# tpfeifle/pointcloud-segmentation-attention

Hardware: AMD Instinct MI355X
Metric: 8192-pt clouds/sec through SA+FP layers, 1/2/4/8 MI355X; HBM GB/s vs peak (higher is better)
Workload: dtype f32

## Files before the change

### include/pn2hip.h

```cpp
#ifndef PN2HIP_H
#define PN2HIP_H

#include <stddef.h>
#include <stdint.h>

#ifdef __cplusplus
extern "C" {
#endif

typedef void* pn2_stream_t;

#define PN2_OK 0
#define PN2_EINVAL (-22)
#define PN2_EFAULT (-14)
#define PN2_ENOTSUP (-95)

#define PN2_FAULT_FPS_POLL 1

#define PN2_FPS_AUTO 0
#define PN2_FPS_BLOCKSCAN 1

#define PN2_USE_XYZ 1
#define PN2_XYZ_LAST 2

// ... 90 lines not shown
  const float* new_xyz;
  int N, C, M, nsample;
  float radius;
  int flags;
  int32_t* idx;
  int32_t* pts_cnt;
  float* grouped_xyz;
  float* new_points;
} pn2_sa_layer;
int pn2_ball_group_layers(const pn2_sa_layer* layers, int nlayers, int B, pn2_stream_t stream);


int pn2_three_nn(const float* xyz1, const float* xyz2, int B, int n, int m, float* dist,
                 int32_t* idx, pn2_stream_t stream);
int pn2_three_interpolate(const float* points, const int32_t* idx, const float* weight, int B,
                          int m, int C, int n, float* out, pn2_stream_t stream);
int pn2_three_interpolate_grad(const float* grad_out, const int32_t* idx, const float* weight,
                               int B, int n, int C, int m, float* grad_points,
                               pn2_stream_t stream);
int pn2cpu_three_nn(const float* xyz1, const float* xyz2, int B, int n, int m, float* dist,
                    int32_t* idx);
int pn2cpu_three_interpolate(const float* points, const int32_t* idx, const float* weight, int B,
                             int m, int C, int n, float* out);
int pn2cpu_three_interpolate_grad(const float* grad_out, const int32_t* idx, const float* weight,
                                  int B, int n, int C, int m, float* grad_points);
int pn2_idw_weights(const float* dist, int B, int n, float* weight, pn2_stream_t stream);
int pn2_fp_fused(const float* xyz1, const float* xyz2, const float* points1, int C1,
                 const float* points2, int C2, int B, int n, int m, float* out,
                 pn2_stream_t stream);

#define PN2_FP_MAX_LAYERS 4
typedef struct pn2_fp_layer {
  const float* xyz1;
  const float* xyz2;
  const float* points1;
  const float* points2;
  int C1, C2, n, m;
  float* out;
} pn2_fp_layer;
int pn2_fp_fused_layers(const pn2_fp_layer* layers, int nlayers, int B, pn2_stream_t stream);

int pn2_three_nn_grid(const void* known_grid, const void* unknown_grid, const float* xyz1,
                      int B, int n, int m, float* dist, int32_t* idx, pn2_stream_t stream);
int pn2_fp_apply(const float* dist, const int32_t* idx, const void* unknown_grid,
                 const float* points1, int C1, const float* points2, int C2, int B, int n, int m,
                 float* out, pn2_stream_t stream);
int pn2_fp_grid_fused(const float* xyz1, const float* xyz2, const void* unknown_grid,
                      const float* points1, int C1, const float* points2, int C2, int B, int n,
                      int m, float* out, float* dist, int32_t* idx, pn2_stream_t stream);
int pn2_fp_grid_fused_known(const void* known_grid, const float* xyz1, const float* xyz2,
                            const void* unknown_grid, const float* points1, int C1,
                            const float* points2, int C2, int B, int n, int m, float* out,
                            float* dist, int32_t* idx, pn2_stream_t stream);


int pn2_attn_reduce(const float* Q, const float* K, const float* V, int B, int M, int ns,
                    int C, float* out, pn2_stream_t stream);
#define PN2_ATTN_MAX_LAYERS 4
typedef struct pn2_attn_layer {
  const float* Q;
  const float* K;
  const float* V;
  int M, ns, C;
  float* out;
} pn2_attn_layer;
int pn2_attn_reduce_layers(const pn2_attn_layer* layers, int nlayers, int B,
                           pn2_stream_t stream);
int pn2_attn_reduce_grad(const float* Q, const float* K, const float* V, const float* grad_out,
                         int B, int M, int ns, int C, float* grad_Q, float* grad_K,
                         float* grad_V, pn2_stream_t stream);
int pn2_group_pool(const float* x, const float* grouped_xyz, int B, int M, int ns, int C,
                   int mode, float* out, pn2_stream_t stream);


size_t pn2_mlp_packed_size(int cin, int cout);
int pn2_mlp_pack(const float* weight, const float* bias, const float* bn_scale,
                 const float* bn_shift, int cin, int cout, void* packed, size_t packed_bytes,
                 pn2_stream_t stream);

int pn2_group_mlp(const float* xyz, const float* points, const float* new_xyz,
                  const int32_t* idx, int B, int N, int C, int M, int nsample, int flags,
                  int nlayers, const pn2_mlp_layer* layers, int pool, float* out,
                  pn2_stream_t stream);
int pn2_group_mlp_attention(const float* xyz, const float* points, const float* new_xyz,
                            const int32_t* idx, int B, int N, int C, int M, int nsample,
                            int flags, int nlayers, const pn2_mlp_layer* layers,
                            const pn2_mlp_layer* qkv, const float* bn_scale,
                            const float* bn_shift, int add_max, float* out,
                            pn2_stream_t stream);
int pn2_fp_mlp(const float* dist, const int32_t* nn_idx, const float* points1, int C1,
               const float* points2, int C2, int B, int n, int m, int nlayers,
               const pn2_mlp_layer* layers, float* out, pn2_stream_t stream);
int pn2_shared_mlp(const float* x, long long rows, int cin, int nlayers,
                   const pn2_mlp_layer* layers, float* out, pn2_stream_t stream);
int pn2_shared_mlp_plan(long long rows, int cin, int nlayers, const pn2_mlp_layer* layers,
                        int* row_tiles, int* tiles_per_wg);


#define PN2_BN_BLOCK_ROWS 1024
size_t pn2_bn_workspace_size(long long rows, int C);
int pn2_bn_stats(const float* y, long long rows, int C, float* mean, float* var, void* workspace,
                 size_t workspace_bytes, pn2_stream_t stream);
int pn2_bn_act_fwd(const float* y, long long rows, int C, const float* mean, const float* var,
                   const float* gamma, const float* beta, float eps, int relu, float* out,
                   pn2_stream_t stream);
int pn2_bn_act_bwd(const float* grad_out, const float* y, long long rows, int C,
// ... 42 lines not shown
```

### pointcloud-segmentation-attention_amd/_lib.py

```python
import ctypes
import os

import torch

_HERE = os.path.dirname(os.path.abspath(__file__))
LIB_PATH = os.environ.get("PN2HIP_LIB") or os.path.join(_HERE, "libpn2hip.so")

PN2_EINVAL = -22
PN2_BQ_MAX_RADII = 3
PN2_EFAULT = -14
PN2_FAULT_FPS_POLL = 1
PN2_ENOTSUP = -95
PN2_FPS_AUTO, PN2_FPS_BLOCKSCAN = 0, 1
PN2_USE_XYZ = 1
PN2_XYZ_LAST = 2
POOL_MODES = {"max": 0, "avg": 1, "weighted_avg": 2, "max_and_avg": 3}
PN2_POOL_NONE = -1
PN2_MLP_MAX_LAYERS = 6
PN2_MLP_RELU = 1


class InvalidArgumentError(ValueError):
    """Raised where the reference's OP_REQUIRES raises tf.errors.InvalidArgumentError."""

# ... 22 lines not shown


class FpLayer(ctypes.Structure):
    _fields_ = [("xyz1", ctypes.c_void_p), ("xyz2", ctypes.c_void_p),
                ("points1", ctypes.c_void_p), ("points2", ctypes.c_void_p), ("C1", ctypes.c_int),
                ("C2", ctypes.c_int), ("n", ctypes.c_int), ("m", ctypes.c_int),
                ("out", ctypes.c_void_p)]


PN2_FP_MAX_LAYERS = 4


class AttnLayer(ctypes.Structure):
    _fields_ = [("Q", ctypes.c_void_p), ("K", ctypes.c_void_p), ("V", ctypes.c_void_p),
                ("M", ctypes.c_int), ("ns", ctypes.c_int), ("C", ctypes.c_int),
                ("out", ctypes.c_void_p)]


PN2_ATTN_MAX_LAYERS = 4

SIGNATURES = {
    "pn2_version": (ctypes.c_char_p, []),
    "pn2_strerror": (ctypes.c_char_p, [_I]),
    "pn2_copy_f4": (_I, [_P, _P, _S, _I, _P]),
    "pn2_fps": (_I, [_P, _I, _I, _I, _P, _P]),
    "pn2_fps_gather": (_I, [_P, _I, _I, _I, _P, _P, _P]),
    "pn2_fps_max_points": (_I, []),
    "pn2_fps_gather_sched": (_I, [_P, _I, _I, _I, _P, _P, _I, _P]),
    "pn2_fault_status": (_I, [_I]),
    "pn2_prob_sample_workspace_size": (_S, [_I, _I]),
    "pn2_prob_sample": (_I, [_P, _P, _I, _I, _I, _P, _S, _P, _P]),
    "pn2_fps_workspace_size": (_S, [_I, _I]),
    "pn2_fps_chain": (_I, [_P, _I, _I, _I, _P, _P, _P, _P]),
    "pn2_fps_chain_grid": (_I, [_P, _I, _I, _I, _P, _P, _P, _P, _S, _P]),
    "pn2_fps_ws": (_I, [_P, _I, _I, _I, _P, _P, _P, _S, _P]),
    "pn2_gather_point": (_I, [_P, _P, _I, _I, _I, _P, _P]),
    "pn2_gather_point_grad": (_I, [_P, _P, _I, _I, _I, _P, _P]),
    "pn2_ball_query": (_I, [_P, _P, _I, _I, _I, _F, _I, _P, _P, _P]),
    "pn2_ball_threshold": (_F, [_F]),
    "pn2_select_top_k": (_I, [_P, _I, _I, _I, _I, _P, _P, _P, _P]),
    "pn2_select_top_k_workspace_size": (_S, [_I, _I, _I]),
    "pn2_knn_point": (_I, [_P, _P, _I, _I, _I, _I, _I, _P, _P, _P]),
    "pn2_grid_size": (_S, [_I, _I]),
    "pn2_grid_build": (_I, [_P, _I, _I, _F, _P, _S, _P]),
    "pn2_ball_query_grid": (_I, [_P, _P, _I, _I, _I, _F, _I, _P, _P, _P]),
    "pn2_ball_group_xyz_grid": (_I, [_P, _P, _P, _I, _I, _I, _F, _I, _P, _P, _P, _P]),
    "pn2_ball_group_grid": (_I, [_P, _P, _P, _I, _I, _P, _I, _I, _I, _F, _I, _P, _P, _P, _P]),
    "pn2_ball_group_xyz_grid_radii": (_I, [_P, _P, _P, _I, _I, _I, _I, _P, _P, _P, _P, _P, _P]),
    "pn2_three_nn_grid": (_I, [_P, _P, _P, _I, _I, _I, _P, _P, _P]),
    "pn2_fp_apply": (_I, [_P, _P, _P, _P, _I, _P, _I, _I, _I, _I, _P, _P]),
    "pn2_fp_grid_fused": (_I, [_P, _P, _P, _P, _I, _P, _I, _I, _I, _I, _P, _P, _P, _P]),
    "pn2_fp_grid_fused_known": (_I, [_P, _P, _P, _P, _P, _I, _P, _I, _I, _I, _I, _P, _P, _P,
                                     _P]),
    "pn2_group_point": (_I, [_P, _P, _I, _I, _I, _I, _I, _P, _P]),
    "pn2_group_point_grad": (_I, [_P, _P, _I, _I, _I, _I, _I, _P, _P]),
    "pn2_group_concat": (_I, [_P, _P, _P, _P, _I, _I, _I, _I, _I, _I, _P, _P, _P]),
    "pn2_ball_group_layers": (_I, [_P, _I, _I, _P]),
    "pn2_sample_and_group": (_I, [_P, _P, _I, _I, _I, _I, _F, _I, _I, _P, _P, _P, _P, _P, _P,
                                  _P]),
    "pn2_three_nn": (_I, [_P, _P, _I, _I, _I, _P, _P, _P]),
    "pn2_three_interpolate": (_I, [_P, _P, _P, _I, _I, _I, _I, _P, _P]),
    "pn2_three_interpolate_grad": (_I, [_P, _P, _P, _I, _I, _I, _I, _P, _P]),
    "pn2_idw_weights": (_I, [_P, _I, _I, _P, _P]),
    "pn2cpu_three_nn": (_I, [_P, _P, _I, _I, _I, _P, _P]),
    "pn2cpu_three_interpolate": (_I, [_P, _P, _P, _I, _I, _I, _I, _P]),
    "pn2cpu_three_interpolate_grad": (_I, [_P, _P, _P, _I, _I, _I, _I, _P]),
    "pn2_fp_fused_layers": (_I, [_P, _I, _I, _P]),
    "pn2_fp_fused": (_I, [_P, _P, _P, _I, _P, _I, _I, _I, _I, _P, _P]),
    "pn2_attn_reduce": (_I, [_P, _P, _P, _I, _I, _I, _I, _P, _P]),
    "pn2_attn_reduce_layers": (_I, [_P, _I, _I, _P]),
    "pn2_attn_reduce_grad": (_I, [_P, _P, _P, _P, _I, _I, _I, _I, _P, _P, _P, _P]),
    "pn2_group_pool": (_I, [_P, _P, _I, _I, _I, _I, _I, _P, _P]),
    "pn2_mlp_packed_size": (_S, [_I, _I]),
    "pn2_mlp_pack": (_I, [_P, _P, _P, _P, _I, _I, _P, _S, _P]),
    "pn2_group_mlp": (_I, [_P, _P, _P, _P, _I, _I, _I, _I, _I, _I, _I, _P, _I, _P, _P]),
    "pn2_group_mlp_attention": (_I, [_P, _P, _P, _P, _I, _I, _I, _I, _I, _I, _I, _P, _P, _P, _P,
                                     _I, _P, _P]),
    "pn2_fp_mlp": (_I, [_P, _P, _P, _I, _P, _I, _I, _I, _I, _I, _P, _P, _P]),
    "pn2_shared_mlp": (_I, [_P, _LL, _I, _I, _P, _P, _P]),
    "pn2_shared_mlp_plan": (_I, [_LL, _I, _I, _P, _P, _P]),
    "pn2_bn_workspace_size": (_S, [_LL, _I]),
    "pn2_bn_stats": (_I, [_P, _LL, _I, _P, _P, _P, _S, _P]),
    "pn2_bn_act_fwd": (_I, [_P, _LL, _I, _P, _P, _P, _P, _F, _I, _P, _P]),
    "pn2_bn_act_bwd": (_I, [_P, _P, _LL, _I, _P, _P, _P, _P, _F, _I, _P, _P, _P, _P, _S, _P]),
    "pn2_bn_act_pool_fwd": (_I, [_P, _LL, _I, _I, _P, _P, _P, _P, _F, _I, _P, _P, _P]),
    "pn2_bn_pool_workspace_size": (_S, [_LL, _I]),
    "pn2_bn_act_pool_bwd": (_I, [_P, _P, _P, _LL, _I, _I, _P, _P, _P, _P, _F, _I, _P, _P, _P, _P,
                                 _S, _P]),
    "pn2_mlp_wgrad_workspace_size": (_S, [_LL, _I, _I]),
    "pn2_mlp_wgrad": (_I, [_P, _P, _LL, _I, _I, _P, _P, _S, _P]),
    "pn2_scene_workspace_size": (_S, [_I]),
    "pn2_scene_bbox": (_I, [_P, _I, _P, _P, _S, _P]),
    "pn2_crop_workspace_size": (_S, [_I, _I, _I]),
    "pn2_crop_sample": (_I, [_P, _P, _P, _P, _I, _P, _P, _I, _I, _P, _I, _P, _I, _P, _S, _P, _P,
                             _P, _P, _P, _P]),
    "pn2_subvolume_slices": (_I, [_I]),
    "pn2_subvolume_select": (_I, [_P, _I, _P, _I, ctypes.c_double, _P, _P, _P, _P]),
    "pn2_gather_rows": (_I, [_P, _LL, _I, _P, _LL, _P, _P]),
    "pn2_plan_create": (_P, []),
    "pn2_plan_destroy": (None, [_P]),
    "pn2_plan_graph": (_I, [_P, _P, _P]),
    "pn2_plan_record": (_I, [_P, _P, _P]),
    "pn2_plan_wait": (_I, [_P, _P, _P]),
    "pn2_plan_fps_chain": (_I, [_P, _P, _I, _I, _I, _P, _P, _P, _P]),
    "pn2_plan_fps_chain_grid": (_I, [_P, _P, _I, _I, _I, _P, _P, _P, _P, _S, _P]),
    "pn2_plan_mark_timed": (_I, [_P]),
# ... 64 lines not shown
```

### pointcloud-segmentation-attention_amd/csrc/interp.hip

```cpp
#include <algorithm>
#include <type_traits>

#include "grid.h"

namespace pn2 {
namespace {

constexpr int kNNBlock = 256;
constexpr int kNNGroup = 4;
constexpr int kNNRows = kNNBlock / kNNGroup;
constexpr int kNNTile = 2048;

struct Best3 {
  float d1, d2, d3;
  int i1, i2, i3;
};

PN2_DEV void best3_init(Best3& b) {
  b.d1 = b.d2 = b.d3 = __builtin_inff();
  b.i1 = b.i2 = b.i3 = 0;
}

PN2_DEV void best3_insert(Best3& b, float d, int k) {
  const bool c1 = d < b.d1, c2 = d < b.d2, c3 = d < b.d3;
// ... 491 lines not shown
      if (ugrid) jj = __float_as_int(grid_view(ugrid, b, n).pts[jj].w);
      s_row[threadIdx.x] = jj;
      const float* D = pdist + ((size_t)b * n + jj) * 3;
      const int32_t* I = pidx + ((size_t)b * n + jj) * 3;
      float w1, w2, w3;
      idw(D[0], D[1], D[2], w1, w2, w3);
      s_idx[threadIdx.x] = make_int4(I[0], I[1], I[2], 0);
      s_w[threadIdx.x] = make_float4(w1, w2, w3, 0.0f);
    }
  } else {
    const int jl = threadIdx.x / kNNGroup;
    const int j = j0 + jl;
    const bool valid = j < n;
    const float* U = xyz1 + ((size_t)b * n + (valid ? j : 0)) * 3;
    Best3 best;
    best3_init(best);
    scan_known(xyz2 + (size_t)b * m * 3, m, U[0], U[1], U[2], sk, best, tile);
    if ((threadIdx.x & (kNNGroup - 1)) == 0) {
      float w1, w2, w3;
      idw(best.d1, best.d2, best.d3, w1, w2, w3);
      s_idx[jl] = make_int4(best.i1, best.i2, best.i3, 0);
      s_w[jl] = make_float4(w1, w2, w3, 0.0f);
    }
  }
  __syncthreads();
  fp_write_rows<V2, V1, UN>(p, b, zb, j0, [&](int rl) {
    if constexpr (PRE) return FpRow{s_idx[rl], s_w[rl], s_row[rl]};
    else return FpRow{s_idx[rl], s_w[rl], j0 + rl};
  });
}

template <int V2, int V1, bool PRE, int UN>
__global__ __launch_bounds__(kNNBlock) void fp_fused_kernel(FpLayer p, int tile) {
  extern __shared__ float4 sk[];
  const int total = (p.n + kNNRows - 1) / kNNRows * p.B * p.Z;
  const int Lg = xcd_block(blockIdx.x, total);
  if (Lg >= total) return;
  fp_fused_body<V2, V1, PRE, UN>(p, Lg, sk, tile);
}

constexpr int kFpGridMaxKnown = 4096;
constexpr float kFpgPointsPerCell = 2.0f;
constexpr int kFpgBlock = 256;
#ifndef PN2_FPG_STAMP
#define PN2_FPG_STAMP 0
#endif
#if PN2_FPG_STAMP
__device__ unsigned long long g_fpg_stamp[4096 * 8];
#define PN2_FPG_T(K) if (t == 0 && Lg < 4096) g_fpg_stamp[Lg * 8 + (K)] = __builtin_amdgcn_s_memtime();
#else
#define PN2_FPG_T(K)
#endif

size_t device_lds_per_block() {
  static size_t cache[64] = {0};
  int dev = 0;
  if (hipGetDevice(&dev) != hipSuccess || dev < 0 || dev >= 64) return 64 * 1024;
  if (!cache[dev]) {
    int v = 0, o = 0;
    if (hipDeviceGetAttribute(&v, hipDeviceAttributeMaxSharedMemoryPerBlock, dev) != hipSuccess)
      v = 0;
    if (hipDeviceGetAttribute(&o, hipDeviceAttributeSharedMemPerBlockOptin, dev) != hipSuccess)
      o = 0;
    v = std::max(v, o);
    if (v <= 0) return 64 * 1024;
    cache[dev] = (size_t)v;
  }
  return cache[dev];
}

inline size_t fp_grid_lds(int m) {
  const size_t cells = (size_t)ceil((double)m * kAutoPointsPerCell / kFpgPointsPerCell);
  return (size_t)m * 16 + ((std::max(cells, (size_t)kAutoMinCells) + 1) * 2 + 3) / 4 * 4;
}

template <int V2, int V1, int UN, int KPT, int FB>
__global__ __launch_bounds__(FB) void fp_grid_fused_kernel(FpLayer p, float* __restrict__ dist,
                                                        int32_t* __restrict__ idx,
                                                        const char* __restrict__ kgrid) {
  constexpr int NW = FB / kWave;
  constexpr int FR = FB / kNNGroup;
  extern __shared__ float4 s_pts[];
  __shared__ int4 s_idx[FR];
  __shared__ float s_wv[3][FR];
  float(*red)[NW] = reinterpret_cast<float(*)[NW]>(&s_wv[0][0]);
  int* wsum = reinterpret_cast<int*>(&s_wv[1][0]);
  GridHdr* shp = reinterpret_cast<GridHdr*>(&s_wv[2][0]);
  static_assert(6 * NW <= FR && sizeof(GridHdr) <= FR * 4, "build scratch fits");
  const int n = p.n, m = p.m;
  const int R = (n + FR - 1) / FR;
  const int total = R * p.B;
  const int Lg = xcd_block(blockIdx.x, total);
  if (Lg >= total) return;
  const int b = Lg / R;
  const int j0 = (Lg - b * R) * FR;
  const int t = threadIdx.x, lane = t & (kWave - 1), w = t / kWave;
  uint16_t* s_off = reinterpret_cast<uint16_t*>(s_pts + m);
  uint32_t* s_cnt = reinterpret_cast<uint32_t*>(s_pts + m);
  PN2_FPG_T(0)
  GridHdr h;
  bool built = false;
  if (kgrid) {
    const char* G = kgrid + (size_t)b * grid_stride(m);
    h = *reinterpret_cast<const GridHdr*>(G);
    if (h.ncell >= 1 && h.ncell <= max(m, kAutoMinCells)) {
      const int* goff = reinterpret_cast<const int*>(G + sizeof(GridHdr));
      const float4* gpts = reinterpret_cast<const float4*>(G + kGridOffBytes);
      for (int i = t; i < m; i += FB) s_pts[i] = gpts[i];
      for (int i = t; i <= h.ncell; i += FB) s_off[i] = (uint16_t)goff[i];
      __syncthreads();
      built = true;
    }
  }
  if (!built) {
    const float* __restrict__ K = p.xyz2 + (size_t)b * m * 3;
    float mn[3] = {INFINITY, INFINITY, INFINITY}, mx[3] = {-INFINITY, -INFINITY, -INFINITY};
#pragma unroll
    for (int i = 0; i < KPT; ++i) {
      const int k = t + i * FB;
      if (k < m) {
#pragma unroll
        for (int a = 0; a < 3; ++a) {
          const float v = K[3 * k + a];
          mn[a] = fminf(mn[a], v);
          mx[a] = fmaxf(mx[a], v);
        }
      }
    }
#pragma unroll
    for (int a = 0; a < 3; ++a) {
      mn[a] = wave_min_f(mn[a]);
      mx[a] = wave_max_f(mx[a]);
    }
    if (lane == 0) {
#pragma unroll
      for (int a = 0; a < 3; ++a) { red[a][w] = mn[a]; red[3 + a][w] = mx[a]; }
    }
    __syncthreads();
    if (t == 0) {
      float lo[3], hi[3];
      for (int a = 0; a < 3; ++a) {
        lo[a] = red[a][0];
        hi[a] = red[3 + a][0];
        for (int i = 1; i < NW; ++i) { lo[a] = fminf(lo[a], red[a][i]); hi[a] = fmaxf(hi[a], red[3 + a][i]); }
        if (!(hi[a] >= lo[a])) { lo[a] = 0.0f; hi[a] = 0.0f; }
      }
      *shp = grid_dims(lo, hi, m, 0.0f, kFpgPointsPerCell);
    }
    __syncthreads();
    h = *shp;
    PN2_FPG_T(1)
    auto cell_at = [&](float x, float y, float z) {
      const int ix = cell_coord(x, h.ox, h.inv, h.nx);
      const int iy = cell_coord(y, h.oy, h.inv, h.ny);
      const int iz = cell_coord(z, h.oz, h.inv, h.nz);
      return (iz * h.ny + iy) * h.nx + ix;
    };

    for (int i = t; i < (h.ncell + 2) / 2; i += FB) s_cnt[i] = 0u;
    __syncthreads();
    int kc[KPT], kr[KPT];
#pragma unroll
    for (int i = 0; i < KPT; ++i) {
      const int k = t + i * FB;
      kc[i] = 0;
      kr[i] = 0;
      if (k < m) {
        const int c = cell_at(K[3 * k + 0], K[3 * k + 1], K[3 * k + 2]);
        const int sh = 16 * (c & 1);
        const uint32_t old = atomicAdd(&s_cnt[c >> 1], 1u << sh);
        kc[i] = c;
        kr[i] = (int)((old >> sh) & 0xFFFFu);
      }
    }
    __syncthreads();
    {
      const int per = (h.ncell + FB - 1) / FB;
      const int s0 = t * per, s1 = min(s0 + per, h.ncell);
      int sum = 0;
      for (int i = s0; i < s1; ++i) sum += s_off[i];
      const int incl = wave_incl_scan(sum, lane);
      if (lane == kWave - 1) wsum[w] = incl;
      __syncthreads();
      int base = incl - sum;
      for (int i = 0; i < w; ++i) base += wsum[i];
      for (int i = s0; i < s1; ++i) {
        const int c = s_off[i];
        s_off[i] = (uint16_t)base;
        base += c;
      }
      if (t == 0) s_off[h.ncell] = (uint16_t)m;
    }
    __syncthreads();
#pragma unroll
    for (int i = 0; i < KPT; ++i) {
      const int k = t + i * FB;
      if (k < m)
        s_pts[s_off[kc[i]] + kr[i]] = make_float4(K[3 * k + 0], K[3 * k + 1], K[3 * k + 2],
                                                  __int_as_float(k));
    }
    __syncthreads();
  }

  PN2_FPG_T(2)
  const int jl = t / kNNGroup, q = t & (kNNGroup - 1);
  const int j = j0 + jl;
  {
    const bool valid = j < n;
    const int jc = valid ? j : n - 1;
    float px, py, pz;
    int u;
    if (p.ugrid) {
      const float4 U = grid_view(p.ugrid, b, n).pts[jc];
      px = U.x; py = U.y; pz = U.z;
      u = __float_as_int(U.w);
    } else {
      const float* U = p.xyz1 + ((size_t)b * n + jc) * 3;
      px = U[0]; py = U[1]; pz = U[2];
      u = jc;
    }
    const Best3 res = grid_nn3_wave<kNNGroup, uint16_t>(h, s_pts, s_off, px, py, pz, q, valid);
    if (valid && q == 0) {
      float w1, w2, w3;
      idw(res.d1, res.d2, res.d3, w1, w2, w3);
      s_idx[jl] = make_int4(res.i1, res.i2, res.i3, u);
      s_wv[0][jl] = w1;
      s_wv[1][jl] = w2;
      s_wv[2][jl] = w3;
      if (dist) {
        float* D = dist + ((size_t)b * n + u) * 3;
        int32_t* I = idx + ((size_t)b * n + u) * 3;
        D[0] = res.d1; D[1] = res.d2; D[2] = res.d3;
        I[0] = res.i1; I[1] = res.i2; I[2] = res.i3;
      }
    }
  }
  __syncthreads();
  PN2_FPG_T(3)
  fp_write_rows<V2, V1, UN, FB>(p, b, 0, j0, [&](int rl) {
    const int4 I = s_idx[rl];
    return FpRow{I, make_float4(s_wv[0][rl], s_wv[1][rl], s_wv[2][rl], 0.0f), I.w};
  });
  PN2_FPG_T(4)
}

constexpr int kFpMaxLayers = PN2_FP_MAX_LAYERS;
struct FpLayers {
  FpLayer l[kFpMaxLayers];
  int first[kFpMaxLayers + 1];
  int nlayers, B;
};
// ... 99 lines not shown
#define PN2_FPG_K(V2, V1, U)                                                                   \
  if (m <= 4 * kFpgBlock) hipLaunchKernelGGL((fp_grid_fused_kernel<V2, V1, U, 4, kFpgBlock>), grid, blk, lds, stream, f.p, dist, idx, kg); \
  else hipLaunchKernelGGL((fp_grid_fused_kernel<V2, V1, U, (kFpGridMaxKnown + kFpgBlock - 1) / kFpgBlock, kFpgBlock>), grid, blk, lds, stream, f.p, dist, idx, kg)
#define PN2_FPG(V2, V1) PN2_FPG_K(V2, V1, kFpUnroll);
  if (f.v1 == 4) { PN2_FPG(4, 4) }
  else if (f.v1 == 2) { PN2_FPG(4, 2) }
  else if (f.v2) { PN2_FPG(4, 1) }
  else { PN2_FPG(1, 1) }
#undef PN2_FPG
#undef PN2_FPG_K
  PN2_RETURN_LAUNCH();
}

int fp_layers_launch(const pn2_fp_layer* layers, int nlayers, int B, hipStream_t stream) {
  if (!layers || nlayers < 1 || nlayers > PN2_FP_MAX_LAYERS || B < 0 || B > 65535)
    return PN2_EINVAL;
  FpLayers a{};
  FpPlan f0{};
  long long blocks = 0;
  int nl = 0, maxm = 0;
  for (int i = 0; i < nlayers; ++i) {
    const pn2_fp_layer& s = layers[i];
    if (s.n < 0 || s.m < 0 || s.C1 < 0 || s.C2 < 0) return PN2_EINVAL;
    if (!s.points1 && s.C1 != 0) return PN2_EINVAL;
    if ((long long)B * s.n == 0 || s.C1 + s.C2 == 0) continue;
    if (!s.xyz1 || !s.out || (s.m > 0 && !s.xyz2) || (s.C2 > 0 && !s.points2)) return PN2_EINVAL;
    if (s.m == 0 && s.C2 > 0) return PN2_EINVAL;
    FpPlan f;
    const int rc = fp_plan(s.xyz1, s.xyz2, nullptr, nullptr, nullptr, s.points1, s.C1,
                                s.points2, s.C2, B, s.n, s.m, s.out, f);
    if (rc != PN2_OK) return rc;
    if (nl == 0) f0 = f;
    if (f.v2 != f0.v2 || f.v1 != f0.v1) {
      PN2_FP_DISPATCH(fp_fused_kernel, f, f.p, f.blocks, s.m, stream);
      const hipError_t e = hipGetLastError();
      if (e != hipSuccess) return (int)e;
      continue;
    }
    a.l[nl] = f.p;
    maxm = std::max(maxm, s.m);
    a.first[nl] = (int)blocks;
    blocks += f.blocks / B;
    ++nl;
  }
  if (nl == 0) return PN2_OK;
  a.first[nl] = (int)blocks;
  a.nlayers = nl;
  a.B = B;
  PN2_FP_DISPATCH(fp_fused_layers_kernel, f0, a, blocks * B, maxm, stream);
  PN2_RETURN_LAUNCH();
}

}
}

extern "C" {

int pn2_three_nn(const float* xyz1, const float* xyz2, int B, int n, int m, float* dist,
                 int32_t* idx, pn2_stream_t stream) {
  if (B < 0 || n < 0 || m < 0 || B > 65535) return PN2_EINVAL;
  if ((long long)B * n == 0) return PN2_OK;
  if (!xyz1 || !dist || !idx || (m > 0 && !xyz2)) return PN2_EINVAL;
  hipLaunchKernelGGL(pn2::three_nn_kernel, dim3((n + pn2::kNNRows - 1) / pn2::kNNRows, B),
                     dim3(pn2::kNNBlock), 0, (hipStream_t)stream, xyz1, xyz2, n, m, dist, idx);
  PN2_RETURN_LAUNCH();
}

int pn2_idw_weights(const float* dist, int B, int n, float* weight, pn2_stream_t stream) {
  if (B < 0 || n < 0) return PN2_EINVAL;
  const long long total = (long long)B * n;
  if (total == 0) return PN2_OK;
  if (total > INT32_MAX || !dist || !weight) return PN2_EINVAL;
  hipLaunchKernelGGL(pn2::idw_kernel, dim3((unsigned)((total + 255) / 256)), dim3(256), 0,
                     (hipStream_t)stream, dist, (int)total, weight);
  PN2_RETURN_LAUNCH();
}

int pn2_three_interpolate(const float* points, const int32_t* idx, const float* weight, int B,
                          int m, int C, int n, float* out, pn2_stream_t stream) {
  if (B < 0 || m < 0 || C < 0 || n < 0) return PN2_EINVAL;
  if ((long long)B * n == 0 || C == 0) return PN2_OK;
  if (!points || !idx || !weight || !out) return PN2_EINVAL;
  const int rows = C >= pn2::kTileElems ? 1 : pn2::kTileElems / C;
  const int chunk = pn2::batch_chunk(B, n, C, rows);
  if (chunk <= 0) return PN2_EINVAL;
  for (int b0 = 0; b0 < B; b0 += chunk) {
    const int nb = B - b0 < chunk ? B - b0 : chunk;
    const long long total_rows = (long long)nb * n;
    const long long tiles = (total_rows + rows - 1) / rows;
    hipLaunchKernelGGL(pn2::three_interp_kernel, dim3((unsigned)tiles), dim3(pn2::kBlock), 0,
                       (hipStream_t)stream, points + (size_t)b0 * m * C, idx + (size_t)b0 * n * 3,
                       weight + (size_t)b0 * n * 3, m, C, n, rows, pn2::make_fastdiv((uint32_t)C),
                       pn2::make_fastdiv((uint32_t)n), (uint32_t)total_rows,
                       out + (size_t)b0 * n * C);
    hipError_t e = hipGetLastError();
    if (e != hipSuccess) return (int)e;
  }
  return PN2_OK;
}

int pn2_three_interpolate_grad(const float* grad_out, const int32_t* idx, const float* weight,
                               int B, int n, int C, int m, float* grad_points,
                               pn2_stream_t stream) {
  if (B < 0 || m < 0 || C < 0 || n < 0) return PN2_EINVAL;
  const size_t bytes = (size_t)B * m * C * sizeof(float);
  if (bytes) {
// ... 58 lines not shown
  if ((dist == nullptr) != (idx == nullptr)) return PN2_EINVAL;
  if ((long long)B * n == 0) return PN2_OK;
  if (C1 + C2 == 0) return dist ? PN2_EINVAL : PN2_OK;
  if (!xyz2 || (!xyz1 && !unknown_grid) || !out || (C2 > 0 && !points2))
    return PN2_EINVAL;
  return pn2::fp_grid_launch(xyz1, xyz2, unknown_grid, points1, C1, points2, C2, B, n, m, out,
                             dist, idx, nullptr, (hipStream_t)stream);
}

#if PN2_FPG_STAMP
int pn2_fpg_stamps(unsigned long long* host_out) {
  return (int)hipMemcpyFromSymbol(host_out, HIP_SYMBOL(pn2::g_fpg_stamp),
                                  sizeof(unsigned long long) * 4096 * 8, 0,
                                  hipMemcpyDeviceToHost);
}
#endif

int pn2_fp_grid_fused_known(const void* known_grid, const float* xyz1, const float* xyz2,
                            const void* unknown_grid, const float* points1, int C1,
                            const float* points2, int C2, int B, int n, int m, float* out,
                            float* dist, int32_t* idx, pn2_stream_t stream) {
  if (!known_grid || ((uintptr_t)known_grid & 15)) return PN2_EINVAL;
  if (B < 0 || n < 0 || m < 1 || m > pn2::kFpGridMaxKnown || C1 < 0 || C2 < 0 || B > 65535)
    return PN2_EINVAL;
  if (!points1 && C1 != 0) return PN2_EINVAL;
  if ((dist == nullptr) != (idx == nullptr)) return PN2_EINVAL;
  if ((long long)B * n == 0) return PN2_OK;
  if (C1 + C2 == 0) return dist ? PN2_EINVAL : PN2_OK;
  if (!xyz2 || (!xyz1 && !unknown_grid) || !out || (C2 > 0 && !points2))
    return PN2_EINVAL;
  return pn2::fp_grid_launch(xyz1, xyz2, unknown_grid, points1, C1, points2, C2, B, n, m, out,
                             dist, idx, known_grid, (hipStream_t)stream);
}

int pn2_three_nn_grid(const void* known_grid, const void* unknown_grid, const float* xyz1,
                      int B, int n, int m, float* dist, int32_t* idx, pn2_stream_t stream) {
  if (B < 0 || n < 0 || m < 0 || B > 65535) return PN2_EINVAL;
  if ((long long)B * n == 0) return PN2_OK;
  if (!known_grid || !dist || !idx || (!unknown_grid && !xyz1)) return PN2_EINVAL;
  constexpr int BLOCK = 256;
  if ((long long)((n + BLOCK / 4 - 1) / (BLOCK / 4)) * B >= (1LL << 31) - 8) return PN2_EINVAL;
  const size_t lds = (size_t)m * 16 + (size_t)(std::max(m, pn2::kAutoMinCells) + 1) * 4;
  constexpr int G = 4, K = 1;
  const dim3 grid(pn2::xcd_grid((long long)((n + BLOCK / G * K - 1) / (BLOCK / G * K)) * B));
  if (lds <= 64 * 1024)
    hipLaunchKernelGGL((pn2::three_nn_grid_kernel<BLOCK, true, G, K>), grid, dim3(BLOCK), lds,
                       (hipStream_t)stream, known_grid, m, unknown_grid, xyz1, n, B, dist, idx);
  else
    hipLaunchKernelGGL((pn2::three_nn_grid_kernel<BLOCK, false, G, K>), grid, dim3(BLOCK), 0,
                       (hipStream_t)stream, known_grid, m, unknown_grid, xyz1, n, B, dist, idx);
  PN2_RETURN_LAUNCH();
}

}
```

### pointcloud-segmentation-attention_amd/csrc/sa_group.hip

```cpp
#include "common.h"

namespace pn2 {
namespace {

constexpr int kSgBlock = 256;
constexpr int kSgWaves = kSgBlock / kWave;
constexpr int kSgCap = 1024;
constexpr int kSgMaxNs = 128;
constexpr int kSgUnroll = 4;
constexpr int kSgHits = 2048;
constexpr int kSgMaxQpb = 64;
constexpr int kSgTileKB = 32;
constexpr int kSgSplitKB = 24;
constexpr int kSgSplitStage = 4096;
constexpr int kSgU = 4;
constexpr int kSgVecFloats = 4096;

enum SgLayout : int {
  PN2_SG_POINTS_ONLY = 0,
  PN2_SG_XYZ_ONLY = 1,
  PN2_SG_XYZ_FIRST = 2,
  PN2_SG_XYZ_LAST = 3,
};

struct SgLayer {
  const float* xyz;
  const float* points;
  const float* new_xyz;
  int32_t* idx;
  int32_t* cnt;
  float* grouped_xyz;
  float* out;
  int N, C, M, ns, Cout, layout, qpb, tiles;
  int parts, chunk;
  int vec;
  float thresh;
  FastDiv div_cout, div_ns, div_c4;
};

struct SgArgs {
  SgLayer l[PN2_SA_MAX_LAYERS];
  int first[PN2_SA_MAX_LAYERS + 1];
  int nlayers, B;
};

PN2_DEV int xyz_channel(int layout, int c, int C, int& cp) {
  cp = c;
  if (layout == PN2_SG_XYZ_ONLY) return c;
  if (layout == PN2_SG_XYZ_FIRST) {
    if (c < 3) return c;
    cp = c - 3;
    return -1;
  }
  if (layout == PN2_SG_XYZ_LAST) return c >= C ? c - C : -1;
  return -1;
}

__global__ __launch_bounds__(kSgBlock) void ball_group_layers_kernel(SgArgs a) {
  __shared__ float sx[kSgCap], sy[kSgCap], sz[kSgCap];
  __shared__ int s_hit[kSgHits];
  __shared__ float s_q[3 * kSgMaxQpb];
  extern __shared__ float4 s_out4[];
  const int per_cloud_all = a.first[a.nlayers];
  const int total = per_cloud_all * a.B;
  const int L = xcd_block((int)blockIdx.x, total);
  if (L >= total) return;
  const int b = L / per_cloud_all;
  const int lc = L - b * per_cloud_all;
  int li = 0;
  while (li + 1 < a.nlayers && lc >= a.first[li + 1]) ++li;
  const SgLayer& g = a.l[li];
  const int local = lc - a.first[li];
  const int tile = local / g.parts;
  const int part = local - tile * g.parts;
  const int t = threadIdx.x, lane = t & (kWave - 1), w = t / kWave;
  const int N = g.N, C = g.C, M = g.M, ns = g.ns, Cout = g.Cout, layout = g.layout;
  const int q0 = tile * g.qpb, nq = min(g.qpb, M - q0);
  const float* __restrict__ P = g.xyz + (size_t)b * N * 3;
  for (int e = t; e < N; e += kSgBlock) {
    sx[e] = P[3 * e + 0];
    sy[e] = P[3 * e + 1];
    sz[e] = P[3 * e + 2];
  }
  const float* __restrict__ Q = g.new_xyz + ((size_t)b * M + q0) * 3;
  for (int e = t; e < 3 * nq; e += kSgBlock) s_q[e] = Q[e];
  __syncthreads();
  const uint64_t lower = (lane == 0) ? 0ull : (~0ull >> (64 - lane));
  for (int qi = w; qi < nq; qi += kSgWaves) {
    const float qx = s_q[3 * qi + 0], qy = s_q[3 * qi + 1], qz = s_q[3 * qi + 2];
    int* hit = s_hit + qi * ns;
    int cnt = 0, first = 0;
    for (int base = 0; base < N && cnt < ns; base += kWave * kSgUnroll) {
      bool h[kSgUnroll];
#pragma unroll
      for (int u = 0; u < kSgUnroll; ++u) {
        const int k = base + u * kWave + lane;
        h[u] = k < N && sqdist(qx, qy, qz, sx[k], sy[k], sz[k]) < g.thresh;
      }
#pragma unroll
      for (int u = 0; u < kSgUnroll; ++u) {
        const uint64_t mask = __ballot(h[u]);
        if (mask != 0ull && cnt < ns) {
          if (cnt == 0) first = base + u * kWave + (__ffsll((unsigned long long)mask) - 1);
          const int pos = cnt + __popcll(mask & lower);
          if (h[u] && pos < ns) hit[pos] = base + u * kWave + lane;
          cnt += __popcll(mask);
        }
      }
    }
    if (cnt > ns) cnt = ns;
    __builtin_amdgcn_fence(__ATOMIC_RELEASE, "wavefront");
    __builtin_amdgcn_wave_barrier();
    __builtin_amdgcn_fence(__ATOMIC_ACQUIRE, "wavefront");
    const size_t gq = (size_t)b * M + q0 + qi;
    int32_t* __restrict__ row = g.idx + gq * ns;
    for (int p = lane; p < ns; p += kWave) {
      const int v = p < cnt ? hit[p] : first;
      hit[p] = v;
      if (part == 0) row[p] = v;
    }
    if (lane == 0 && part == 0) g.cnt[gq] = cnt;
  }
  __syncthreads();
  const size_t r_base = ((size_t)b * M + q0) * ns;
  float* __restrict__ O = g.out + r_base * Cout;
  float* __restrict__ GX = g.grouped_xyz ? g.grouped_xyz + r_base * 3 : nullptr;
  const float* __restrict__ F = g.points ? g.points + (size_t)b * N * C : nullptr;
  if (g.vec) {
    {
      float* s_out = reinterpret_cast<float*>(s_out4);
      const int C4 = C >> 2;
      const int foff = layout == PN2_SG_XYZ_FIRST ? 3 : 0;
      const int xoff = layout == PN2_SG_XYZ_LAST ? C : 0;
      const bool has_xyz = layout != PN2_SG_POINTS_ONLY;
      const int CH = (kSgVecFloats / Cout) & ~3;
      const int R = nq * ns;
      const int RP = (((R + g.parts - 1) / g.parts) + 3) & ~3;
      const int rbeg = part * RP, rend = min(R, rbeg + RP);
      const float4* __restrict__ F4 = reinterpret_cast<const float4*>(F);
      constexpr int UV = 4;
      float4 v[UV];
      int dst[UV];
      auto gather = [&](int c0, int f0) {
        const int nf = min(CH, rend - c0) * C4;
#pragma unroll
        for (int u = 0; u < UV; ++u) {
          const int f = min(f0 + u * kSgBlock, nf - 1);
          const int rr = (int)fdiv((uint32_t)f, g.div_c4);
          const int cc = f - rr * C4;
          v[u] = F4[(size_t)s_hit[c0 + rr] * C4 + cc];
          dst[u] = rr * Cout + foff + 4 * cc;
        }
      };
      const bool one_pass = CH * C4 <= kSgBlock * UV;
      if (one_pass && rbeg < rend) gather(rbeg, t);
      for (int c0 = rbeg; c0 < rend; c0 += CH) {
        const int nr = min(CH, rend - c0);
        const int nf = nr * C4;
        for (int f0 = t; f0 < nf; f0 += kSgBlock * UV) {
          if (!one_pass) gather(c0, f0);
#pragma unroll
          for (int u = 0; u < UV; ++u) {
            if (f0 + u * kSgBlock < nf) {
              s_out[dst[u]] = v[u].x;
              s_out[dst[u] + 1] = v[u].y;
              s_out[dst[u] + 2] = v[u].z;
              s_out[dst[u] + 3] = v[u].w;
            }
          }
        }
        if (has_xyz) {
          for (int e = t; e < nr * 3; e += kSgBlock) {
            const int rr = e / 3, cx = e - 3 * rr;
            const int r = c0 + rr;
            const int qi = (int)fdiv((uint32_t)r, g.div_ns);
            const int i = s_hit[r];
            const float sv = cx == 0 ? sx[i] : (cx == 1 ? sy[i] : sz[i]);
            s_out[rr * Cout + xoff + cx] = sv - s_q[3 * qi + cx];
          }
        }
        __syncthreads();
        if (one_pass && c0 + CH < rend) gather(c0 + CH, t);
        float4* __restrict__ O4 = reinterpret_cast<float4*>(O + (size_t)c0 * Cout);
        const int n4 = (nr * Cout) >> 2;
        for (int k = t; k < n4; k += kSgBlock) O4[k] = s_out4[k];
        __syncthreads();
      }
      return;
    }
  }
  const int e_beg = part * g.chunk;
  const int E = min(nq * ns * Cout, e_beg + g.chunk);
  auto value = [&](int e) -> float {
    const int r = (int)fdiv((uint32_t)e, g.div_cout);
    const int c = e - r * Cout;
    const int qi = (int)fdiv((uint32_t)r, g.div_ns);
    const int i = s_hit[r];
    int cp;
    const int cx = xyz_channel(layout, c, C, cp);
    if (cx >= 0) {
      const float s = cx == 0 ? sx[i] : (cx == 1 ? sy[i] : sz[i]);
      const float v = s - s_q[3 * qi + cx];
      if (GX) GX[(size_t)r * 3 + cx] = v;
      return v;
    }
    return F[(size_t)i * C + cp];
  };
  constexpr int U = kSgU;
  for (int e0 = e_beg + t; e0 < E; e0 += kSgBlock * U) {
    float v[U];
#pragma unroll
    for (int u = 0; u < U; ++u) {
      const int e = e0 + u * kSgBlock;
      v[u] = e < E ? value(e) : 0.0f;
    }
#pragma unroll
    for (int u = 0; u < U; ++u) {
      const int e = e0 + u * kSgBlock;
      if (e < E) O[e] = v[u];
    }
  }
  if (GX && layout == PN2_SG_POINTS_ONLY && part == 0) {
    for (int e = t; e < nq * ns * 3; e += kSgBlock) {
      const int r = e / 3, cx = e - 3 * (e / 3);
      const int qi = (int)fdiv((uint32_t)r, g.div_ns);
      const int i = s_hit[r];
      const float s = cx == 0 ? sx[i] : (cx == 1 ? sy[i] : sz[i]);
      GX[e] = s - s_q[3 * qi + cx];
    }
  }
}

}
}

extern "C" {

int pn2_ball_group_layers(const pn2_sa_layer* layers, int nlayers, int B, pn2_stream_t stream) {
  if (!layers || nlayers < 1 || nlayers > PN2_SA_MAX_LAYERS || B < 0 || B > 65535)
    return PN2_EINVAL;
  pn2::SgArgs a{};
  a.nlayers = nlayers;
  long long blocks = 0;
  for (int i = 0; i < nlayers; ++i) {
    const pn2_sa_layer& s = layers[i];
    pn2::SgLayer& g = a.l[i];
    if (!(s.radius > 0.0f) || s.nsample <= 0 || s.nsample > pn2::kSgMaxNs || s.N < 0 ||
        s.N > pn2::kSgCap || s.M < 0 || s.C < 0)
      return PN2_EINVAL;
    using namespace pn2;
    int layout, Cout;
    if (!s.points || s.C == 0) { layout = PN2_SG_XYZ_ONLY; Cout = 3; }
    else if (!(s.flags & PN2_USE_XYZ)) { layout = PN2_SG_POINTS_ONLY; Cout = s.C; }
    else { layout = (s.flags & PN2_XYZ_LAST) ? PN2_SG_XYZ_LAST : PN2_SG_XYZ_FIRST; Cout = s.C + 3; }
    if ((long long)B * s.M > 0) {
      if (!s.xyz || !s.new_xyz || !s.idx || !s.pts_cnt || !s.new_points) return PN2_EINVAL;
      if (s.N == 0) return PN2_EINVAL;
    }
    g.xyz = s.xyz;
    g.points = layout == PN2_SG_XYZ_ONLY ? nullptr : s.points;
    g.new_xyz = s.new_xyz;
    g.idx = s.idx;
    g.cnt = s.pts_cnt;
    g.grouped_xyz = s.grouped_xyz;
    g.out = s.new_points;
    g.N = s.N; g.C = layout == PN2_SG_XYZ_ONLY ? 0 : s.C; g.M = s.M; g.ns = s.nsample;
    g.Cout = Cout; g.layout = layout;
    g.thresh = pn2_ball_threshold(s.radius);
    g.div_cout = pn2::make_fastdiv((uint32_t)Cout);
    const long long per_q = (long long)s.nsample * Cout * 4;
    long long qpb = (kSgTileKB * 1024 + per_q / 2) / per_q;
    if (qpb < 1) qpb = 1;
    if (qpb > pn2::kSgMaxQpb) qpb = pn2::kSgMaxQpb;
    if (qpb * s.nsample > pn2::kSgHits) qpb = pn2::kSgHits / s.nsample;
    long long parts = 1;
    if (s.N * 12 <= kSgSplitStage && per_q > kSgSplitKB * 1024) {
      qpb = 1;
      parts = (per_q + kSgSplitKB * 1024 - 1) / (kSgSplitKB * 1024);
    }
    const long long E = qpb * s.nsample * Cout;
    g.chunk = (int)(((E + parts - 1) / parts + 3) / 4 * 4);
    g.parts = (int)((E + g.chunk - 1) / g.chunk);
    if (E * (long long)Cout >= (1LL << 32)) return PN2_EINVAL;
    g.qpb = (int)qpb;
    g.div_ns = pn2::make_fastdiv((uint32_t)s.nsample);
    g.tiles = s.M > 0 ? (int)((s.M + qpb - 1) / qpb) : 0;
    g.div_c4 = pn2::make_fastdiv((uint32_t)(s.C / 4 > 0 ? s.C / 4 : 1));
    g.vec = layout != PN2_SG_XYZ_ONLY && s.C % 4 == 0 && s.nsample % 4 == 0 &&
            !s.grouped_xyz && 4 * Cout <= pn2::kSgVecFloats &&
            (((uintptr_t)s.points | (uintptr_t)s.new_points) & 15) == 0;
    a.first[i] = (int)blocks;
    blocks += (long long)g.tiles * g.parts;
    if (blocks * B >= (1LL << 31) - 8) return PN2_EINVAL;
  }
  a.first[nlayers] = (int)blocks;
  a.B = B;
  if (blocks * B == 0) return PN2_OK;
  bool vec = false;
  for (int i = 0; i < nlayers; ++i) vec = vec || a.l[i].vec;
  const size_t lds = vec ? (size_t)pn2::kSgVecFloats * 4 : 0;
  hipLaunchKernelGGL(pn2::ball_group_layers_kernel, dim3(pn2::xcd_grid(blocks * B)),
                     dim3(pn2::kSgBlock), lds, (hipStream_t)stream, a);
  PN2_RETURN_LAUNCH();
}

}
```

Baseline: 98140.

## Cut LDS and register pressure in FP grid and SA grouping kernels

The FP grid kernel gains an occupancy hint (waves_per_eu 8), makes the grid header wave-uniform so it can live in scalar registers, and packs each point's cell and rank into one 32-bit register. The SA grouping kernel aliases the xyz cloud arrays onto the output staging buffer in a single static LDS allocation, stores hit indices as 16-bit values, and prefetches centred xyz values from global memory during the overlapped gather. An occupancy reporting API is added for inspection. The waves_per_eu hint risks register spills, and reading xyz from global rather than LDS may add latency.

```diff
diff --git a/include/pn2hip.h b/include/pn2hip.h
--- a/include/pn2hip.h
+++ b/include/pn2hip.h
@@ -166,6 +166,10 @@
                             const void* unknown_grid, const float* points1, int C1,
                             const float* points2, int C2, int B, int n, int m, float* out,
                             float* dist, int32_t* idx, pn2_stream_t stream);
+
+#define PN2_OCC_FP4 0
+#define PN2_OCC_SA_GROUP 1
+int pn2_occupancy_report(int kernel, int* out);
 
 
 int pn2_attn_reduce(const float* Q, const float* K, const float* V, int B, int M, int ns,
diff --git a/pointcloud-segmentation-attention_amd/_lib.py b/pointcloud-segmentation-attention_amd/_lib.py
--- a/pointcloud-segmentation-attention_amd/_lib.py
+++ b/pointcloud-segmentation-attention_amd/_lib.py
@@ -98,6 +98,7 @@
     "pn2_fp_grid_fused": (_I, [_P, _P, _P, _P, _I, _P, _I, _I, _I, _I, _P, _P, _P, _P]),
     "pn2_fp_grid_fused_known": (_I, [_P, _P, _P, _P, _P, _I, _P, _I, _I, _I, _I, _P, _P, _P,
                                      _P]),
+    "pn2_occupancy_report": (_I, [_I, _P]),
     "pn2_group_point": (_I, [_P, _P, _I, _I, _I, _I, _I, _P, _P]),
     "pn2_group_point_grad": (_I, [_P, _P, _I, _I, _I, _I, _I, _P, _P]),
     "pn2_group_concat": (_I, [_P, _P, _P, _P, _I, _I, _I, _I, _I, _I, _P, _P, _P]),
diff --git a/pointcloud-segmentation-attention_amd/csrc/interp.hip b/pointcloud-segmentation-attention_amd/csrc/interp.hip
--- a/pointcloud-segmentation-attention_amd/csrc/interp.hip
+++ b/pointcloud-segmentation-attention_amd/csrc/interp.hip
@@ -567,6 +567,19 @@
 #define PN2_FPG_T(K)
 #endif
 
+PN2_DEV GridHdr uniform_hdr(const GridHdr& v) {
+  GridHdr h;
+  h.ox = __uint_as_float(uniform_u32(__float_as_uint(v.ox)));
+  h.oy = __uint_as_float(uniform_u32(__float_as_uint(v.oy)));
+  h.oz = __uint_as_float(uniform_u32(__float_as_uint(v.oz)));
+  h.inv = __uint_as_float(uniform_u32(__float_as_uint(v.inv)));
+  h.nx = (int)uniform_u32((uint32_t)v.nx);
+  h.ny = (int)uniform_u32((uint32_t)v.ny);
+  h.nz = (int)uniform_u32((uint32_t)v.nz);
+  h.ncell = (int)uniform_u32((uint32_t)v.ncell);
+  return h;
+}
+
 size_t device_lds_per_block() {
   static size_t cache[64] = {0};
   int dev = 0;
@@ -590,9 +603,9 @@
 }
 
 template <int V2, int V1, int UN, int KPT, int FB>
-__global__ __launch_bounds__(FB) void fp_grid_fused_kernel(FpLayer p, float* __restrict__ dist,
-                                                        int32_t* __restrict__ idx,
-                                                        const char* __restrict__ kgrid) {
+__global__ __launch_bounds__(FB) __attribute__((amdgpu_waves_per_eu(8, 8)))
+void fp_grid_fused_kernel(FpLayer p, float* __restrict__ dist, int32_t* __restrict__ idx,
+                          const char* __restrict__ kgrid) {
   constexpr int NW = FB / kWave;
   constexpr int FR = FB / kNNGroup;
   extern __shared__ float4 s_pts[];
@@ -663,7 +676,7 @@
       *shp = grid_dims(lo, hi, m, 0.0f, kFpgPointsPerCell);
     }
     __syncthreads();
-    h = *shp;
+    h = uniform_hdr(*shp);
     PN2_FPG_T(1)
     auto cell_at = [&](float x, float y, float z) {
       const int ix = cell_coord(x, h.ox, h.inv, h.nx);
@@ -674,18 +687,16 @@
 
     for (int i = t; i < (h.ncell + 2) / 2; i += FB) s_cnt[i] = 0u;
     __syncthreads();
-    int kc[KPT], kr[KPT];
+    uint32_t kcr[KPT];
 #pragma unroll
     for (int i = 0; i < KPT; ++i) {
       const int k = t + i * FB;
-      kc[i] = 0;
-      kr[i] = 0;
+      kcr[i] = 0u;
       if (k < m) {
         const int c = cell_at(K[3 * k + 0], K[3 * k + 1], K[3 * k + 2]);
         const int sh = 16 * (c & 1);
         const uint32_t old = atomicAdd(&s_cnt[c >> 1], 1u << sh);
-        kc[i] = c;
-        kr[i] = (int)((old >> sh) & 0xFFFFu);
+        kcr[i] = ((uint32_t)c << 16) | ((old >> sh) & 0xFFFFu);
       }
     }
     __syncthreads();
@@ -711,7 +722,7 @@
     for (int i = 0; i < KPT; ++i) {
       const int k = t + i * FB;
       if (k < m)
-        s_pts[s_off[kc[i]] + kr[i]] = make_float4(K[3 * k + 0], K[3 * k + 1], K[3 * k + 2],
+        s_pts[s_off[kcr[i] >> 16] + (kcr[i] & 0xFFFFu)] = make_float4(K[3 * k + 0], K[3 * k + 1], K[3 * k + 2],
                                                   __int_as_float(k));
     }
     __syncthreads();
@@ -917,6 +928,7 @@
 }
 
 }
+int sg_occupancy(int* out);
 }
 
 extern "C" {
@@ -1081,4 +1093,25 @@
   PN2_RETURN_LAUNCH();
 }
 
-}
+int pn2_occupancy_report(int kernel, int* out) {
+  if (!out) return PN2_EINVAL;
+  if (kernel == PN2_OCC_SA_GROUP) return pn2::sg_occupancy(out);
+  if (kernel != PN2_OCC_FP4) return PN2_EINVAL;
+  const void* fn = reinterpret_cast<const void*>(
+      &pn2::fp_grid_fused_kernel<4, 4, pn2::kFpUnroll, 4, pn2::kFpgBlock>);
+  const size_t lds = pn2::fp_grid_lds(1024);
+  hipFuncAttributes at;
+  hipError_t e = hipFuncGetAttributes(&at, fn);
+  if (e != hipSuccess) return (int)e;
+  int nb = 0;
+  e = hipOccupancyMaxActiveBlocksPerMultiprocessor(&nb, fn, pn2::kFpgBlock, lds);
+  if (e != hipSuccess) return (int)e;
+  out[0] = nb;
+  out[1] = at.numRegs;
+  out[2] = (int)at.sharedSizeBytes;
+  out[3] = (int)lds;
+  out[4] = (int)at.localSizeBytes;
+  return PN2_OK;
+}
+
+}
diff --git a/pointcloud-segmentation-attention_amd/csrc/sa_group.hip b/pointcloud-segmentation-attention_amd/csrc/sa_group.hip
--- a/pointcloud-segmentation-attention_amd/csrc/sa_group.hip
+++ b/pointcloud-segmentation-attention_amd/csrc/sa_group.hip
@@ -10,7 +10,10 @@
 constexpr int kSgUnroll = 4;
 constexpr int kSgHits = 2048;
 constexpr int kSgMaxQpb = 64;
-constexpr int kSgTileKB = 32;
+#ifndef PN2_SG_TILE_KB
+#define PN2_SG_TILE_KB 32
+#endif
+constexpr int kSgTileKB = PN2_SG_TILE_KB;
 constexpr int kSgSplitKB = 24;
 constexpr int kSgSplitStage = 4096;
 constexpr int kSgU = 4;
@@ -57,10 +60,15 @@
 }
 
 __global__ __launch_bounds__(kSgBlock) void ball_group_layers_kernel(SgArgs a) {
-  __shared__ float sx[kSgCap], sy[kSgCap], sz[kSgCap];
-  __shared__ int s_hit[kSgHits];
+  __shared__ float4 s_raw4[kSgVecFloats / 4];
+  static_assert(3 * kSgCap <= kSgVecFloats, "the cloud fits the chunk image's array");
+  float* const sx = reinterpret_cast<float*>(s_raw4);
+  float* const sy = sx + kSgCap;
+  float* const sz = sy + kSgCap;
+  float4* const s_out4 = s_raw4;
+  __shared__ uint16_t s_hit[kSgHits];
+  static_assert(kSgCap <= 65536, "a hit (a point of the cloud) fits 16 bits");
   __shared__ float s_q[3 * kSgMaxQpb];
-  extern __shared__ float4 s_out4[];
   const int per_cloud_all = a.first[a.nlayers];
   const int total = per_cloud_all * a.B;
   const int L = xcd_block((int)blockIdx.x, total);
@@ -88,7 +96,7 @@
   const uint64_t lower = (lane == 0) ? 0ull : (~0ull >> (64 - lane));
   for (int qi = w; qi < nq; qi += kSgWaves) {
     const float qx = s_q[3 * qi + 0], qy = s_q[3 * qi + 1], qz = s_q[3 * qi + 2];
-    int* hit = s_hit + qi * ns;
+    uint16_t* hit = s_hit + qi * ns;
     int cnt = 0, first = 0;
     for (int base = 0; base < N && cnt < ns; base += kWave * kSgUnroll) {
       bool h[kSgUnroll];
@@ -103,7 +111,7 @@
         if (mask != 0ull && cnt < ns) {
           if (cnt == 0) first = base + u * kWave + (__ffsll((unsigned long long)mask) - 1);
           const int pos = cnt + __popcll(mask & lower);
-          if (h[u] && pos < ns) hit[pos] = base + u * kWave + lane;
+          if (h[u] && pos < ns) hit[pos] = (uint16_t)(base + u * kWave + lane);
           cnt += __popcll(mask);
         }
       }
@@ -116,7 +124,7 @@
     int32_t* __restrict__ row = g.idx + gq * ns;
     for (int p = lane; p < ns; p += kWave) {
       const int v = p < cnt ? hit[p] : first;
-      hit[p] = v;
+      hit[p] = (uint16_t)v;
       if (part == 0) row[p] = v;
     }
     if (lane == 0 && part == 0) g.cnt[gq] = cnt;
@@ -153,7 +161,19 @@
         }
       };
       const bool one_pass = CH * C4 <= kSgBlock * UV;
+      auto centred = [&](int c0, int e) -> float {
+        const int rr = e / 3, cx = e - 3 * rr;
+        const int r = c0 + rr;
+        const int qi = (int)fdiv((uint32_t)r, g.div_ns);
+        return P[3 * (int)s_hit[r] + cx] - s_q[3 * qi + cx];
+      };
+      const bool xpre = one_pass && has_xyz && CH * 3 <= kSgBlock;
+      float xv = 0.0f;
+      auto xfetch = [&](int c0) {
+        if (t < min(CH, rend - c0) * 3) xv = centred(c0, t);
+      };
       if (one_pass && rbeg < rend) gather(rbeg, t);
+      if (xpre && rbeg < rend) xfetch(rbeg);
       for (int c0 = rbeg; c0 < rend; c0 += CH) {
         const int nr = min(CH, rend - c0);
         const int nf = nr * C4;
@@ -169,18 +189,17 @@
             }
           }
         }
-        if (has_xyz) {
+        if (xpre) {
+          if (t < nr * 3) s_out[(t / 3) * Cout + xoff + (t - 3 * (t / 3))] = xv;
+        } else if (has_xyz) {
           for (int e = t; e < nr * 3; e += kSgBlock) {
             const int rr = e / 3, cx = e - 3 * rr;
-            const int r = c0 + rr;
-            const int qi = (int)fdiv((uint32_t)r, g.div_ns);
-            const int i = s_hit[r];
-            const float sv = cx == 0 ? sx[i] : (cx == 1 ? sy[i] : sz[i]);
-            s_out[rr * Cout + xoff + cx] = sv - s_q[3 * qi + cx];
+            s_out[rr * Cout + xoff + cx] = centred(c0, e);
           }
         }
         __syncthreads();
         if (one_pass && c0 + CH < rend) gather(c0 + CH, t);
+        if (xpre && c0 + CH < rend) xfetch(c0 + CH);
         float4* __restrict__ O4 = reinterpret_cast<float4*>(O + (size_t)c0 * Cout);
         const int n4 = (nr * Cout) >> 2;
         for (int k = t; k < n4; k += kSgBlock) O4[k] = s_out4[k];
@@ -199,7 +218,7 @@
     int cp;
     const int cx = xyz_channel(layout, c, C, cp);
     if (cx >= 0) {
-      const float s = cx == 0 ? sx[i] : (cx == 1 ? sy[i] : sz[i]);
+      const float s = sx[cx * kSgCap + i];
       const float v = s - s_q[3 * qi + cx];
       if (GX) GX[(size_t)r * 3 + cx] = v;
       return v;
@@ -225,13 +244,30 @@
       const int r = e / 3, cx = e - 3 * (e / 3);
       const int qi = (int)fdiv((uint32_t)r, g.div_ns);
       const int i = s_hit[r];
-      const float s = cx == 0 ? sx[i] : (cx == 1 ? sy[i] : sz[i]);
+      const float s = sx[cx * kSgCap + i];
       GX[e] = s - s_q[3 * qi + cx];
     }
   }
 }
 
 }
+
+int sg_occupancy(int* out) {
+  const void* fn = reinterpret_cast<const void*>(&ball_group_layers_kernel);
+  hipFuncAttributes at;
+  hipError_t e = hipFuncGetAttributes(&at, fn);
+  if (e != hipSuccess) return (int)e;
+  int nb = 0;
+  e = hipOccupancyMaxActiveBlocksPerMultiprocessor(&nb, fn, kSgBlock, 0);
+  if (e != hipSuccess) return (int)e;
+  out[0] = nb;
+  out[1] = at.numRegs;
+  out[2] = (int)at.sharedSizeBytes;
+  out[3] = 0;
+  out[4] = (int)at.localSizeBytes;
+  return PN2_OK;
+}
+
 }
 
 extern "C" {
@@ -296,11 +332,8 @@
   a.first[nlayers] = (int)blocks;
   a.B = B;
   if (blocks * B == 0) return PN2_OK;
-  bool vec = false;
-  for (int i = 0; i < nlayers; ++i) vec = vec || a.l[i].vec;
-  const size_t lds = vec ? (size_t)pn2::kSgVecFloats * 4 : 0;
   hipLaunchKernelGGL(pn2::ball_group_layers_kernel, dim3(pn2::xcd_grid(blocks * B)),
-                     dim3(pn2::kSgBlock), lds, (hipStream_t)stream, a);
+                     dim3(pn2::kSgBlock), 0, (hipStream_t)stream, a);
   PN2_RETURN_LAUNCH();
 }
 
```

Result: no change. 98680, median of 6 (+0.5%).
